# barbararoessle/e2e_multi_view_matching

Measured on AMD Instinct MI355X. Metric: image-pairs/sec @1024 kpts + pose AUC@5/10/20deg vs reference, higher is better.
Workload: dtype f16x2 (fp32 operands carried as 2 fp16 planes hi + 2^-11 lo', 22 significant bits, 3 fp16-MFMA products, fp32 accumulate; same 1e-4 / bit-exact-index parity bar); 1 GPU; configs[1]: tuple_size=2 (1 pair per tuple), 1024 keypoints, 256-dim f32 descriptors, GNN 9x1 = 18 layers, 100 Sinkhorn iters, batch 32 tuples/GPU = 32 pairs/GPU, w8pt pose per pair; pairs_per_gpu=32, global_pairs=32, weights=random init (timed), identity-like for the AUC leg, parallelism=tuple-sharded x1

## Files before the change

e2e_multi_view_matching_amd/csrc/attention_p2w.hip:

```cpp
#include <algorithm>
#include <type_traits>

#include "attention_p2.h"

namespace e2emv {

typedef __attribute__((ext_vector_type(16))) float aw_f32x16;

constexpr int AW_QT = 256;
constexpr int AW_TILEB = 64 * 256;
constexpr int AW_REGB = 2 * AW_TILEB;
constexpr int AW_PART_F = 68;
constexpr float AW_SINV = 1.f / P2_QS, AW_PLOG = 7.f, AW_LIMIT = 60000.f;

__device__ __forceinline__ void aw_wait_q(p2_f16x8 (&q)[2][2][4]) {
    asm volatile("s_waitcnt vmcnt(16)"
                 : "+a"(q[0][0][0]), "+a"(q[0][0][1]), "+a"(q[0][0][2]), "+a"(q[0][0][3]), "+a"(q[0][1][0]), "+a"(q[0][1][1]), "+a"(q[0][1][2]), "+a"(q[0][1][3]),
                   "+a"(q[1][0][0]), "+a"(q[1][0][1]), "+a"(q[1][0][2]), "+a"(q[1][0][3]), "+a"(q[1][1][0]), "+a"(q[1][1][1]), "+a"(q[1][1][2]), "+a"(q[1][1][3])
                 :: "memory");
}

template <int I, int N, class F>
__device__ __forceinline__ void aw_for(F&& f) {
    if constexpr (I < N) {
        f(std::integral_constant<int, I>{});
        aw_for<I + 1, N>(f);
    }
}

__device__ __forceinline__ unsigned aw_cvt_pk(float v0, float v1) {
    const p2_f32x2 vv = {v0, v1};
    return __builtin_bit_cast(unsigned, __builtin_convertvector(vv, p2_f16x2));
}
__device__ __forceinline__ float aw_fma(float a, float b, float c) {
    float d;
    asm volatile("v_fma_f32 %0, %1, %2, %3" : "=v"(d) : "v"(a), "v"(b), "v"(c));
    return d;
}
__device__ __forceinline__ float aw_exp2(float a) {
    float d;
    asm volatile("v_exp_f32 %0, %1" : "=v"(d) : "v"(a));
    return d;
}
__device__ __forceinline__ void aw_acc(float& sum, float a) { asm volatile("v_add_f32 %0, %0, %1" : "+v"(sum) : "v"(a)); }
__device__ __forceinline__ unsigned aw_cvt_pk_v(float v0, float v1) {
    unsigned d;
    asm volatile("v_cvt_pk_f16_f32 %0, %1, %2" : "=v"(d) : "v"(v0), "v"(v1));
    return d;
}
__device__ __forceinline__ unsigned aw_mixlo(unsigned hi, float v0) {
    unsigned lo;
    asm volatile("v_fma_mixlo_f16 %0, %1, -1.0, %2 op_sel_hi:[1,0,0]" : "=v"(lo) : "v"(hi), "v"(v0));
    return lo;
}
__device__ __forceinline__ unsigned aw_mixhi(unsigned lo, unsigned hi, float v1) {
    asm volatile("v_fma_mixhi_f16 %0, %1, -1.0, %2 op_sel:[1,0,0] op_sel_hi:[1,0,0]" : "+v"(lo) : "v"(hi), "v"(v1));
    return lo;
}
__device__ __forceinline__ unsigned aw_lo(unsigned hi, float v0, float v1) {
    unsigned lo;
    asm("v_fma_mixlo_f16 %0, %1, -1.0, %2 op_sel_hi:[1,0,0]\n\tv_fma_mixhi_f16 %0, %1, -1.0, %3 op_sel:[1,0,0] op_sel_hi:[1,0,0]"
        : "=&v"(lo) : "v"(hi), "v"(v0), "v"(v1));
    return lo;
}

__device__ __forceinline__ void aw_mfma_s(aw_f32x16& c, p2_f16x8 a, p2_f16x8 b) {
    asm volatile("v_mfma_f32_32x32x16_f16 %0, %1, %2, %0" : "+v"(c) : "v"(a), "a"(b));
}
__device__ __forceinline__ void aw_mfma_s0(aw_f32x16& c, p2_f16x8 a, p2_f16x8 b) {
    asm volatile("v_mfma_f32_32x32x16_f16 %0, %1, %2, 0" : "=&v"(c) : "v"(a), "a"(b));
}
__device__ __forceinline__ void aw_mfma_sa(aw_f32x16& c, p2_f16x8 a, p2_f16x8 b) {
    asm volatile("v_mfma_f32_32x32x16_f16 %0, %1, %2, %0" : "+v"(c) : "a"(a), "a"(b));
}
__device__ __forceinline__ void aw_mfma_sa0(aw_f32x16& c, p2_f16x8 a, p2_f16x8 b) {
    asm volatile("v_mfma_f32_32x32x16_f16 %0, %1, %2, 0" : "=&v"(c) : "a"(a), "a"(b));
}
__device__ __forceinline__ void aw_mfma_oa(aw_f32x16& c, p2_f16x8 a, p2_u32x4 b) {
    asm volatile("v_mfma_f32_32x32x16_f16 %0, %1, %2, %0" : "+a"(c) : "a"(a), "v"(b));
}
template <int IMM>
__device__ __forceinline__ void aw_read_frag(p2_f16x8& d, unsigned addr) {
    static_assert(IMM >= 0 && IMM < 65536, "ds_read offset: 16 bits");
    asm volatile("ds_read_b128 %0, %1 offset:%2" : "=a"(d) : "v"(addr), "n"(IMM));
}
template <int N>
__device__ __forceinline__ void aw_wait_frag(p2_f16x8 (&f)[4]) {
    asm volatile("s_waitcnt lgkmcnt(%4)" : "+a"(f[0]), "+a"(f[1]), "+a"(f[2]), "+a"(f[3]) : "n"(N));
}
__device__ __forceinline__ void aw_load_q(const char* qp, p2_f16x8 (&q)[2][4]) {
    asm volatile(
        "global_load_dwordx4 %0, %8, off\n\t"
        "global_load_dwordx4 %1, %8, off offset:32\n\t"
        "global_load_dwordx4 %2, %8, off offset:128\n\t"
        "global_load_dwordx4 %3, %8, off offset:160\n\t"
        "global_load_dwordx4 %4, %8, off offset:64\n\t"
        "global_load_dwordx4 %5, %8, off offset:96\n\t"
        "global_load_dwordx4 %6, %8, off offset:192\n\t"
        "global_load_dwordx4 %7, %8, off offset:224"
        : "=&a"(q[0][0]), "=&a"(q[0][1]), "=&a"(q[0][2]), "=&a"(q[0][3]), "=&a"(q[1][0]), "=&a"(q[1][1]), "=&a"(q[1][2]), "=&a"(q[1][3])
        : "v"(qp) : "memory");
}

template <bool HAS_E, bool MULTI = true, bool PART = false>
__global__ __launch_bounds__(256, 1) void attention_p2w_kernel(AttnP2Params p) {
    extern __shared__ __attribute__((aligned(16))) char smem_aw[];

    int lin = blockIdx.x, ks = 0;
    constexpr bool part = PART;
    if constexpr (PART) {
        const int h = blockIdx.x, tpx = (8 * p.gper * p.nq - p.n_full) >> 3;
        ks = (h >> 3) / tpx;
        lin = p.n_full + 8 * ((h >> 3) % tpx) + (h & 7);
    }
    const int xcd = lin & 7, idx = lin >> 3;
    const int g = xcd * p.gper + idx / p.nq;
    if (g >= p.groups) return;
    const int qt = idx % p.nq;
    const int img = g / p.H, head = g % p.H;
    const int b = img / p.T, t = img % p.T;
    if (qt * AW_QT >= p.nv[t]) return;

    const int tid = threadIdx.x, lane = tid & 63;
    const int wave = __builtin_amdgcn_readfirstlane(tid >> 6);
    const int l31 = lane & 31, lh = lane >> 5;
    const unsigned row_b = 8u * (unsigned)p.D;

    int q_row[2];
    bool q_ok[2];
    p2_f16x8 Qf[2][2][4];
#pragma unroll
    for (int a = 0; a < 2; ++a) {
        q_row[a] = qt * AW_QT + wave * 64 + a * 32 + l31;
        q_ok[a] = q_row[a] < p.n_rows;
        const char* qp = reinterpret_cast<const char*>(p.qk) + ((int64_t)img * p.n_rows + (q_ok[a] ? q_row[a] : p.n_rows - 1)) * row_b + head * 256;
        aw_load_q(qp + lh * 16, Qf[a]);
    }
    const int q_blk = __builtin_amdgcn_readfirstlane(((int64_t)img * p.n_rows + min(qt * AW_QT + wave * 64, p.n_rows - 1)) >> 6);
    const int e_q = HAS_E ? p.EQK[q_blk * 8 + head] : 0;

    const int n_src = p.cross ? p.T - 1 : 1;
    auto src_t = [&](int si) __attribute__((always_inline)) { return !p.cross ? t : (si < t ? si : si + 1); };
    int n_tiles = 0;
    for (int si = 0; si < n_src; ++si) n_tiles += (p.nv[src_t(si)] + 63) / 64;
    int t0 = 0;
    if constexpr (PART) {
        t0 = ks * n_tiles / p.n_split;
        n_tiles = (ks + 1) * n_tiles / p.n_split - t0;
        if (n_tiles <= 0) return;
    }
    struct Cur { int si, kt, nv; unsigned kb, vb; int eb; };
    auto cur_src = [&](Cur& c) __attribute__((always_inline)) {
        const int im = b * p.T + src_t(c.si);
        c.kt = 0;
        c.nv = p.nv[src_t(c.si)];
        c.kb = (unsigned)(im * p.n_rows) * row_b;
        c.vb = (unsigned)((im * p.H + head) * 64) * (unsigned)p.n_rows * 4u;
        c.eb = (im * p.n_rows) >> 6;
    };
    auto cur_next = [&](Cur& c) __attribute__((always_inline)) {
        ++c.kt;
        if constexpr (MULTI) {
            if (c.kt * 64 >= c.nv && c.si + 1 < n_src) { ++c.si; cur_src(c); }
        }
    };
    auto cur_init = [&]() __attribute__((always_inline)) {
        Cur c;
        c.si = 0;
        cur_src(c);
        if constexpr (PART)
            for (int i = 0; i < t0; ++i) cur_next(c);
        return c;
    };

    const __amdgpu_buffer_rsrc_t rsK = __builtin_amdgcn_make_buffer_rsrc(const_cast<uint16_t*>(p.qk), 0, (int)p.qk_bytes, 0x00020000);
    const __amdgpu_buffer_rsrc_t rsV = __builtin_amdgcn_make_buffer_rsrc(const_cast<uint16_t*>(p.vt), 0, (int)p.vt_bytes, 0x00020000);
    unsigned k_vo[4], v_vo[4];
#pragma unroll
    for (int i = 0; i < 4; ++i) {
        const int row = 4 * (wave * 4 + i) + (lane >> 4);
        const unsigned c = (unsigned)((lane & 15) ^ (row & 15));
        k_vo[i] = (unsigned)row * row_b + 4u * (unsigned)p.D + (unsigned)head * 256u + c * 16u;
        v_vo[i] = (unsigned)row * (unsigned)p.n_rows * 4u + c * 16u;
    }
    auto k_so = [&](const Cur& c) __attribute__((always_inline)) { return c.kb + (unsigned)c.kt * 64u * row_b; };
    auto v_so = [&](const Cur& c) __attribute__((always_inline)) { return c.vb + (unsigned)c.kt * 256u; };
    auto k_piece = [&](int region, int i, unsigned so) __attribute__((always_inline)) { p2_glds16(rsK, smem_aw + region * AW_REGB + AW_TILEB + (wave * 4 + i) * 1024, k_vo[i], so); };
    auto v_piece = [&](int region, int i, unsigned so) __attribute__((always_inline)) { p2_glds16(rsV, smem_aw + region * AW_REGB + (wave * 4 + i) * 1024, v_vo[i], so); };
    int* const els = reinterpret_cast<int*>(smem_aw + 3 * AW_REGB);
    int ek_mine = 0, ev_mine = 0;
    if (HAS_E && tid < n_tiles) {
        int si = 0, kt = PART ? tid + t0 : tid;
        if constexpr (MULTI) {
            for (; si + 1 < n_src; ++si) {
                const int nt = (p.nv[src_t(si)] + 63) / 64;
                if (kt < nt) break;
                kt -= nt;
            }
        }
        const int blk = (((b * p.T + src_t(si)) * p.n_rows) >> 6) + kt;
        ek_mine = p.EQK[blk * 8 + 4 + head];
        if (p.EVt) ev_mine = p.EVt[blk * 4 + head];
    }
    typedef __attribute__((address_space(3))) const p2_u32x2* lds_pair_t;
    const unsigned els0 = (unsigned)(uintptr_t)(__attribute__((address_space(3))) char*)smem_aw + 3u * AW_REGB;
    auto read_e = [&](int tl) __attribute__((always_inline)) {
        return *reinterpret_cast<lds_pair_t>((uintptr_t)(els0 + 8u * (unsigned)min(tl, n_tiles - 1)));
    };

    const int kz = l31 & 15;
    const unsigned lds0 = (unsigned)(uintptr_t)(__attribute__((address_space(3))) char*)smem_aw;
    unsigned R[4][2];
#pragma unroll
    for (int s = 0; s < 4; ++s)
#pragma unroll
        for (int pl = 0; pl < 2; ++pl)
            R[s][pl] = lds0 + (unsigned)(l31 * 256 + ((((s >> 1) * 8 + pl * 4 + 2 * (s & 1) + lh) ^ kz) << 4));
    typedef __attribute__((address_space(3))) const p2_f16x8* lds_frag_t;
    auto frag = [&](int s, int pl, int imm) __attribute__((always_inline)) { return *reinterpret_cast<lds_frag_t>((uintptr_t)(R[s][pl] + (unsigned)imm)); };

    constexpr int PA[3] = {1, 0, 0};
    constexpr int PB[3] = {0, 1, 0};

    aw_f32x16 O[2][2], S[2][2];
    p2_u32x4 Pf[2][2][4];
#pragma unroll
    for (int a = 0; a < 2; ++a)
#pragma unroll
        for (int d = 0; d < 2; ++d)
#pragma unroll
            for (int r = 0; r < 16; ++r) O[a][d][r] = 0.f;
    float m_run[2] = {-1e30f, -1e30f}, l_run[2] = {0.f, 0.f};
    int e_o = 0;
    bool o_started = false;
    unsigned n_slow = 0;

    auto sm_slow = [&](auto BB, float sinv, int valid) __attribute__((always_inline)) {
        constexpr int B = decltype(BB)::value;
        asm volatile("s_nop 15" : "+v"(S[B][0]), "+v"(S[B][1]), "+a"(O[B][0]), "+a"(O[B][1]));
        if (valid < 64) {
#pragma unroll
            for (int kb = 0; kb < 2; ++kb)
#pragma unroll
                for (int r = 0; r < 16; ++r)
                    if (kb * 32 + (r & 3) + 8 * (r >> 2) + 4 * lh >= valid) S[B][kb][r] = -INFINITY;
        }
        float mx = S[B][0][0];
#pragma unroll
        for (int kb = 0; kb < 2; ++kb)
#pragma unroll
            for (int r = 0; r < 16; ++r) mx = fmaxf(mx, S[B][kb][r]);
        {
            float x = mx, y = mx;
            asm volatile("s_nop 1\n\tv_permlane32_swap_b32 %0, %1\n\ts_nop 1" : "+v"(x), "+v"(y));
            mx = fmaxf(x, y);
        }
        mx *= sinv;
        const float m_new = fmaxf(m_run[B], mx);
        const float alpha = __builtin_amdgcn_exp2f(m_run[B] - m_new);
#pragma unroll
        for (int r = 0; r < 16; ++r) { O[B][0][r] *= alpha; O[B][1][r] *= alpha; }
        const float e0 = AW_PLOG - m_new;
        float ps = 0.f;
#pragma unroll
        for (int k = 0; k < 16; ++k) {
            const int kb = k >> 3, r = 2 * (k & 7), u = 2 * kb + ((k & 7) >> 2), e = k & 3;
            const float p0 = __builtin_amdgcn_exp2f(__builtin_fmaf(S[B][kb][r], sinv, e0));
            const float p1 = __builtin_amdgcn_exp2f(__builtin_fmaf(S[B][kb][r + 1], sinv, e0));
            ps += p0 + p1;
            const P2Pair pr = p2_split_plain(p0, p1);
            Pf[B][0][u][e] = pr.hi; Pf[B][1][u][e] = pr.lo;
        }
        l_run[B] = l_run[B] * alpha + ps;
        m_run[B] = m_new;
        asm volatile("s_nop 4" : "+a"(O[B][0]), "+a"(O[B][1]));
    };

    Cur cK = cur_init(), cV = cur_init(), cS = cur_init();
    int nK = 0, nV = 0;
    auto adv_k = [&]() __attribute__((always_inline)) { if (++nK < n_tiles) cur_next(cK); };
    auto adv_v = [&]() __attribute__((always_inline)) { if (++nV < n_tiles) cur_next(cV); };
    {
        const unsigned so = k_so(cK);
#pragma unroll
        for (int i = 0; i < 4; ++i) k_piece(2, i, so);
        adv_k();
    }
#pragma unroll
    for (int r = 0; r < 2; ++r) {
        const unsigned sov = v_so(cV), sok = k_so(cK);
#pragma unroll
        for (int i = 0; i < 4; ++i) v_piece(r, i, sov);
#pragma unroll
        for (int i = 0; i < 4; ++i) k_piece(r, i, sok);
        adv_v();
        adv_k();
    }
    if (HAS_E && tid < n_tiles) { els[2 * tid] = ek_mine; els[2 * tid + 1] = ev_mine; }
    aw_wait_q(Qf);
    __syncthreads();
    p2_u32x2 e_pair = {0u, 0u};
    if constexpr (HAS_E) e_pair = read_e(0);
#pragma unroll
    for (int s = 0; s < 4; ++s)
#pragma unroll
        for (int pl = 0; pl < 2; ++pl) R[s][pl] += 2 * AW_REGB;
    {
        const float sinv = AW_SINV * p2_exp2i(e_q + __builtin_amdgcn_readfirstlane((int)e_pair[0]));
#pragma unroll
        for (int a = 0; a < 2; ++a)
#pragma unroll
            for (int s = 0; s < 4; ++s) {
                p2_f16x8 kf[2][2];
#pragma unroll
                for (int kb = 0; kb < 2; ++kb)
#pragma unroll
                    for (int pl = 0; pl < 2; ++pl) kf[kb][pl] = frag(s, pl, AW_TILEB + kb * 8192);
#pragma unroll
                for (int q = 0; q < 3; ++q)
#pragma unroll
                    for (int kb = 0; kb < 2; ++kb) {
                        if (s == 0 && q == 0) aw_mfma_s0(S[a][kb], kf[kb][PA[q]], Qf[a][PB[q]][s]);
                        else aw_mfma_s(S[a][kb], kf[kb][PA[q]], Qf[a][PB[q]][s]);
                    }
            }
        asm volatile("s_waitcnt vmcnt(8) lgkmcnt(0)\n\ts_barrier" ::: "memory");
        sm_slow(std::integral_constant<int, 0>{}, sinv, cS.nv - cS.kt * 64);
        if (cS.nv - cS.kt * 64 >= 64) {
            asm volatile("s_nop 15" : "+v"(S[1][0]), "+v"(S[1][1]));
            float mx = S[1][0][0];
#pragma unroll
            for (int kb = 0; kb < 2; ++kb)
#pragma unroll
                for (int r = 0; r < 16; ++r) mx = fmaxf(mx, S[1][kb][r]);
            float x = mx, y = mx;
            asm volatile("s_nop 1\n\tv_permlane32_swap_b32 %0, %1\n\ts_nop 1" : "+v"(x), "+v"(y));
            m_run[1] = fmaxf(x, y) * sinv;
        }
    }
#pragma unroll
    for (int s = 0; s < 4; ++s)
#pragma unroll
        for (int pl = 0; pl < 2; ++pl) R[s][pl] -= 2 * AW_REGB;
    int reg_cur = 0, seg_tile = 0;

    p2_f16x8 FA[8][4];
    auto read_frag = [&](auto GG, auto NN, auto SS, auto KK) __attribute__((always_inline)) {
        constexpr int G = decltype(GG)::value, N = decltype(NN)::value, S = decltype(SS)::value, KPART = decltype(KK)::value;
        constexpr int x = N & 1, pl = N < 2 ? 1 : 0;
        aw_read_frag<KPART * AW_TILEB + x * 8192>(FA[G][N], R[S][pl]);
    };
    aw_for<0, 8>([&](auto II) __attribute__((always_inline)) {
        constexpr int g = decltype(II)::value / 4, n = decltype(II)::value % 4;
        read_frag(std::integral_constant<int, g>{}, std::integral_constant<int, n>{}, std::integral_constant<int, g>{}, std::integral_constant<int, 0>{});
    });

    auto seg = [&](auto AA, auto LL) __attribute__((always_inline)) {
        constexpr int A = decltype(AA)::value, B = 1 - A;
        constexpr bool LAST = decltype(LL)::value;
        constexpr bool HAS_SM = !(LAST && A == 1);
        constexpr int NSLOT = LAST ? 24 : 48, NG = NSLOT / 6;
        constexpr int MPS = LAST ? 2 : 1;

        if (A == 0) {
            if (HAS_E && p.EVt) {
                const int e_v = __builtin_amdgcn_readfirstlane((int)e_pair[1]);
                if (__builtin_expect(o_started && e_v != e_o, 0)) {
                    const float f = e_o - e_v < -126 ? 0.f : p2_exp2i(e_o - e_v);
                    asm volatile("s_nop 15" : "+a"(O[0][0]), "+a"(O[0][1]), "+a"(O[1][0]), "+a"(O[1][1]));
#pragma unroll
                    for (int a = 0; a < 2; ++a)
#pragma unroll
                        for (int r = 0; r < 16; ++r) { O[a][0][r] *= f; O[a][1][r] *= f; }
                    asm volatile("s_nop 4" : "+a"(O[0][0]), "+a"(O[0][1]), "+a"(O[1][0]), "+a"(O[1][1]));
                }
                e_o = e_v;
                o_started = true;
            }
        }
        float sinv = AW_SINV, e0 = 0.f, ps = 0.f;
        int valid = 64;
        if (HAS_SM) {
            if (HAS_E) sinv = AW_SINV * p2_exp2i(e_q + __builtin_amdgcn_readfirstlane((int)e_pair[0]));
            if (HAS_E && A == 0 && !LAST) e_pair = read_e(seg_tile + 1);
            e0 = AW_PLOG - m_run[B];
            valid = cS.nv - cS.kt * 64;
        }
        if (HAS_SM && __builtin_expect(valid < 64, 0)) {
            asm volatile("s_nop 7" : "+v"(S[B][0]), "+v"(S[B][1]));
#pragma unroll
            for (int kb = 0; kb < 2; ++kb)
#pragma unroll
                for (int r = 0; r < 16; ++r)
                    if (kb * 32 + (r & 3) + 8 * (r >> 2) + 4 * lh >= valid) S[B][kb][r] = -INFINITY;
            asm volatile("" : "+v"(S[B][0]), "+v"(S[B][1]));
        }
        bool slow = false;
        float xa[16][2], pa[16][2], psA = 0.f, psB = 0.f, sinv_v = sinv;
        asm volatile("" : "+v"(sinv_v), "+v"(e0));
        unsigned hi_k[16], lo_k[16];
        auto micro = [&](auto MM) __attribute__((always_inline)) {
            constexpr int m = decltype(MM)::value;
            constexpr int k = m / 3, ph = m % 3;
            constexpr int kb = (k & 15) >> 3, r = 2 * (k & 7);
            if constexpr (m == 48) {
                lo_k[15] = aw_mixlo(hi_k[15], pa[15][0]);
            } else if constexpr (m == 49) {
                Pf[B][1][3][3] = aw_mixhi(lo_k[15], hi_k[15], pa[15][1]);
            } else if constexpr (ph == 0) {
                xa[k][0] = aw_fma(S[B][kb][r], sinv_v, e0);
                if constexpr (k > 0) lo_k[k - 1] = aw_mixlo(hi_k[k - 1], pa[k - 1][0]);
                xa[k][1] = aw_fma(S[B][kb][r + 1], sinv_v, e0);
            } else if constexpr (ph == 1) {
                pa[k][0] = aw_exp2(xa[k][0]);
                if constexpr (k > 0) {
                    constexpr int k1 = k - 1, u = 2 * (k1 >> 3) + ((k1 & 7) >> 2), e = k1 & 3;
                    Pf[B][1][u][e] = aw_mixhi(lo_k[k1], hi_k[k1], pa[k1][1]);
                }
                pa[k][1] = aw_exp2(xa[k][1]);
            } else {
                constexpr int u = 2 * (k >> 3) + ((k & 7) >> 2), e = k & 3;
                aw_acc(psA, pa[k][0]);
                hi_k[k] = aw_cvt_pk_v(pa[k][0], pa[k][1]);
                Pf[B][0][u][e] = hi_k[k];
                aw_acc(psB, pa[k][1]);
            }
        };

        unsigned so_v = 0, so_k = 0;
        if (A == 0 && !LAST) {
            so_v = v_so(cV);
            adv_v();
            so_k = k_so(cK);
            adv_k();
        }
        const int reg_ld = reg_cur == 0 ? 2 : reg_cur - 1;

        aw_for<0, NSLOT>([&](auto II) __attribute__((always_inline)) {
            constexpr int i = decltype(II)::value;
            constexpr int gq = i / 6, w = i % 6;
            if constexpr (A == 0 && w == 0) aw_wait_frag<(gq + 1 < NG ? 4 : 0)>(FA[gq]);
            if constexpr (i < 24) {
                constexpr int u = i / 6, q = (i % 6) / 2, db = i % 2;
                aw_mfma_oa(O[A][db], FA[u][db + 2 * (1 - PA[q])], Pf[A][PB[q]][u]);
            } else {
                constexpr int s = (i - 24) / 6, q = (i % 6) / 2, kb = i % 2;
                if constexpr (s == 0 && q == 0) aw_mfma_sa0(S[A][kb], FA[4 + s][kb + 2 * (1 - PA[q])], Qf[A][PB[q]][s]);
                else aw_mfma_sa(S[A][kb], FA[4 + s][kb + 2 * (1 - PA[q])], Qf[A][PB[q]][s]);
            }
            if constexpr (HAS_SM) {
                if constexpr (LAST) {
                    aw_for<0, MPS>([&](auto JJ) __attribute__((always_inline)) { micro(std::integral_constant<int, MPS * i + decltype(JJ)::value>{}); });
                } else if constexpr (i < 9) {
                    constexpr int m0 = i + i / 2 - (i > 0 && i % 2 == 0 ? 1 : 0);
                    micro(std::integral_constant<int, m0>{});
                    if constexpr (i >= 2 && i % 2 == 0) micro(std::integral_constant<int, m0 + 1>{});
                } else if constexpr (i < 46) {
                    micro(std::integral_constant<int, i + 4>{});
                } else if constexpr (i == 46) {
                    ps = psA;
                    aw_acc(ps, psB);
                } else if constexpr (i == 47) {
                    slow = __builtin_amdgcn_ballot_w64(!(ps < AW_LIMIT)) != 0;
                    l_run[B] += slow ? 0.f : ps;
                }
            }
            if constexpr (A == 1 && !LAST && i == 36) {
                asm volatile("s_waitcnt vmcnt(8) lgkmcnt(0)\n\ts_barrier" ::: "memory");
                const unsigned d = reg_cur == 2 ? (unsigned)(-2 * AW_REGB) : (unsigned)AW_REGB;
#pragma unroll
                for (int s = 0; s < 4; ++s)
#pragma unroll
                    for (int pl = 0; pl < 2; ++pl) R[s][pl] += d;
                reg_cur = reg_cur == 2 ? 0 : reg_cur + 1;
            }
            if constexpr (w >= 1 && w <= 4) {
                constexpr int gn = gq + 2;
                constexpr auto N = std::integral_constant<int, w - 1>{};
                if constexpr (A == 0 && gn < NG) {
                    if constexpr (gn < 4) read_frag(std::integral_constant<int, gn>{}, N, std::integral_constant<int, gn>{}, std::integral_constant<int, 0>{});
                    else read_frag(std::integral_constant<int, gn>{}, N, std::integral_constant<int, gn - 4>{}, std::integral_constant<int, 1>{});
                } else if constexpr (A == 1 && !LAST && gn >= NG) {
                    read_frag(std::integral_constant<int, gn - NG>{}, N, std::integral_constant<int, gn - NG>{}, std::integral_constant<int, 0>{});
                }
            }
            if constexpr (A == 0 && !LAST && i < 32 && i % 4 == 1) {
                if constexpr (i < 16) v_piece(reg_ld, i / 4, so_v);
                else k_piece(reg_ld, i / 4 - 4, so_k);
            }
            __builtin_amdgcn_sched_barrier(0);
        });

        if constexpr (HAS_SM && LAST) {
            lo_k[15] = aw_mixlo(hi_k[15], pa[15][0]);
            ps = psA + psB;
            Pf[B][1][3][3] = aw_mixhi(lo_k[15], hi_k[15], pa[15][1]);
            const bool slow = __builtin_amdgcn_ballot_w64(!(ps < AW_LIMIT)) != 0;
            l_run[B] += slow ? 0.f : ps;
            if (__builtin_expect(slow, 0)) {
                sm_slow(std::integral_constant<int, B>{}, sinv, valid);
                ++n_slow;
            }
        }
        if constexpr (HAS_SM && !LAST) {
            if (__builtin_expect(slow, 0)) {
                sm_slow(std::integral_constant<int, B>{}, sinv, valid);
                ++n_slow;
            }
        }
        if (A == 0) cur_next(cS);
    };

    for (int j = 0; j + 1 < n_tiles; ++j) {
        seg_tile = j;
        seg(std::integral_constant<int, 0>{}, std::false_type{});
        seg(std::integral_constant<int, 1>{}, std::false_type{});
    }
    seg(std::integral_constant<int, 0>{}, std::true_type{});
    seg(std::integral_constant<int, 1>{}, std::true_type{});

    asm volatile("s_waitcnt vmcnt(0)" ::: "memory");
    asm volatile("s_nop 15" : "+a"(O[0][0]), "+a"(O[0][1]), "+a"(O[1][0]), "+a"(O[1][1]));
    if constexpr (PART) {
        const int64_t rec = ((int64_t)(lin - p.n_full) * p.n_split + ks) * AW_QT;
        if (lane == 0) p.part_e[rec / 64 + wave] = e_o;
#pragma unroll
        for (int a = 0; a < 2; ++a) {
            const float l_tot = l_run[a] + __shfl_xor(l_run[a], 32);
            float* o = p.part + (rec + wave * 64 + a * 32 + l31) * AW_PART_F;
#pragma unroll
            for (int d = 0; d < 2; ++d)
#pragma unroll
                for (int gq = 0; gq < 4; ++gq)
                    *reinterpret_cast<p2_f32x4*>(o + 32 * d + 8 * gq + 4 * lh) = p2_f32x4{O[a][d][4 * gq], O[a][d][4 * gq + 1], O[a][d][4 * gq + 2], O[a][d][4 * gq + 3]};
            if (lh == 0) { o[64] = m_run[a]; o[65] = l_tot; }
        }
        if (p.stats && n_slow && lane == 0) atomicAdd(p.stats, n_slow);
        return;
    }
    if (p.EO && lane == 0 && q_ok[0]) p.EO[(((int64_t)img * p.n_rows + q_row[0]) >> 6) * 4 + head] = e_o;
#pragma unroll
    for (int a = 0; a < 2; ++a) {
        const float l_tot = l_run[a] + __shfl_xor(l_run[a], 32);
        const float inv = 1.f / (l_tot * P2_VS);
        uint16_t* op = p.out + p2_index((int64_t)img * p.n_rows + q_row[a], head * 64, p.D) + 8 * lh;
#pragma unroll
        for (int d = 0; d < 2; ++d)
#pragma unroll
            for (int kp = 0; kp < 2; ++kp) {
                const int r0 = 8 * kp, r1 = 8 * kp + 4;
                const P2Pair x0 = p2_split_scaled(O[a][d][r0] * inv, O[a][d][r0 + 1] * inv), x1 = p2_split_scaled(O[a][d][r0 + 2] * inv, O[a][d][r0 + 3] * inv);
                const P2Pair y0 = p2_split_scaled(O[a][d][r1] * inv, O[a][d][r1 + 1] * inv), y1 = p2_split_scaled(O[a][d][r1 + 2] * inv, O[a][d][r1 + 3] * inv);
                const auto h0 = __builtin_amdgcn_permlane32_swap(x0.hi, y0.hi, false, false), h1 = __builtin_amdgcn_permlane32_swap(x1.hi, y1.hi, false, false);
                const auto l0 = __builtin_amdgcn_permlane32_swap(x0.lo, y0.lo, false, false), l1 = __builtin_amdgcn_permlane32_swap(x1.lo, y1.lo, false, false);
                uint16_t* o = op + d * 64 + kp * 16;
                if (q_ok[a]) {
                    *reinterpret_cast<p2_u32x4*>(o) = p2_u32x4{h0[0], h1[0], h0[1], h1[1]};
                    *reinterpret_cast<p2_u32x4*>(o + 32) = p2_u32x4{l0[0], l1[0], l0[1], l1[1]};
                }
            }
    }
    if (p.stats && n_slow && lane == 0) atomicAdd(p.stats, n_slow);
}

__global__ __launch_bounds__(1024) void attention_p2w_combine(AttnP2Params p) {
    const int item = blockIdx.x, lin = p.n_full + item;
    const int xcd = lin & 7, idx = lin >> 3;
    const int g = xcd * p.gper + idx / p.nq;
    if (g >= p.groups) return;
    const int qt = idx % p.nq, img = g / p.H, head = g % p.H, t = img % p.T;
    if (qt * AW_QT >= p.nv[t]) return;
    const int n_src = p.cross ? p.T - 1 : 1;
    int n_tiles = 0;
    for (int si = 0; si < n_src; ++si) n_tiles += (p.nv[!p.cross ? t : (si < t ? si : si + 1)] + 63) / 64;
    const int q = threadIdx.x >> 2, dq = (threadIdx.x & 3) * 16;
    const int row = qt * AW_QT + q;
    float m = -3.0e38f;
    int e = -1000;
    for (int k = 0; k < p.n_split; ++k) {
        if ((k + 1) * n_tiles / p.n_split - k * n_tiles / p.n_split <= 0) continue;
        const int64_t rec = ((int64_t)item * p.n_split + k) * AW_QT;
        m = fmaxf(m, p.part[(rec + q) * AW_PART_F + 64]);
        e = max(e, p.part_e[rec / 64 + (q >> 6)]);
    }
    float acc[16], l = 0.f;
#pragma unroll
    for (int i = 0; i < 16; ++i) acc[i] = 0.f;
    for (int k = 0; k < p.n_split; ++k) {
        if ((k + 1) * n_tiles / p.n_split - k * n_tiles / p.n_split <= 0) continue;
        const int64_t rec = ((int64_t)item * p.n_split + k) * AW_QT;
        const float* o = p.part + (rec + q) * AW_PART_F;
        const int ek = p.part_e[rec / 64 + (q >> 6)];
        const float a = __builtin_amdgcn_exp2f(o[64] - m);
        const float ae = a * (ek - e < -126 ? 0.f : p2_exp2i(ek - e));
        l += a * o[65];
#pragma unroll
        for (int i = 0; i < 16; i += 4) {
            const p2_f32x4 v = *reinterpret_cast<const p2_f32x4*>(o + dq + i);
            acc[i] += ae * v[0]; acc[i + 1] += ae * v[1]; acc[i + 2] += ae * v[2]; acc[i + 3] += ae * v[3];
        }
    }
    if (row >= p.n_rows) return;
    if (p.EO && (threadIdx.x & 255) == 0) p.EO[(((int64_t)img * p.n_rows + row) >> 6) * 4 + head] = e;
    const float inv = 1.f / (l * P2_VS);
    uint16_t* op = p.out + p2_index((int64_t)img * p.n_rows + row, head * 64 + dq, p.D);
#pragma unroll
    for (int h = 0; h < 2; ++h) {
        p2_u32x4 hi, lo;
#pragma unroll
        for (int i = 0; i < 4; ++i) {
            const P2Pair pr = p2_split_scaled(acc[8 * h + 2 * i] * inv, acc[8 * h + 2 * i + 1] * inv);
            hi[i] = pr.hi; lo[i] = pr.lo;
        }
        *reinterpret_cast<p2_u32x4*>(op + 8 * h) = hi;
        *reinterpret_cast<p2_u32x4*>(op + 8 * h + 32) = lo;
    }
}

int launch_attention_p2w(e2emv_ctx* ctx, AttnP2Params& p, int n_valid, hipStream_t s) {
    p.nq = (n_valid + AW_QT - 1) / AW_QT;
    if (int rc = ensure_flags(ctx)) return rc;
    p.stats = ctx->d_flags + 5;
    const size_t lds = 3 * AW_REGB + 2048;
    const bool multi = p.cross && p.T > 2;
    const void* fn = p.EQK ? (multi ? reinterpret_cast<const void*>(attention_p2w_kernel<true, true>) : reinterpret_cast<const void*>(attention_p2w_kernel<true, false>))
                           : (multi ? reinterpret_cast<const void*>(attention_p2w_kernel<false, true>) : reinterpret_cast<const void*>(attention_p2w_kernel<false, false>));
    if (int rc = ensure_dynamic_lds(ctx, fn, lds)) return rc;
    void* args[] = {&p};
    const int n_items = 8 * p.gper * p.nq, cus = std::max(8, ctx->num_cus / 8 * 8);
    const int r = n_items % cus;
    const int min_tiles = attn_min_tiles(p, 64);
    p.n_full = n_items;
    p.n_split = 1;
    p.part = nullptr;
    p.part_e = nullptr;
    if (ctx->attn_key_split && r > 0 && 2 * r <= cus && r % 8 == 0) {
        const int k = std::min(std::min(cus / r, 8), min_tiles);
        if (k >= 2) {
            const size_t n_rec = (size_t)r * k * AW_QT;
            const size_t need = n_rec * AW_PART_F * sizeof(float) + (n_rec / 64) * sizeof(int);
            if (need > ctx->attn_part_bytes) {
                if (ctx->d_attn_part) { E2EMV_HIP(ctx, hipStreamSynchronize(s)); (void)hipFree(ctx->d_attn_part); ctx->d_attn_part = nullptr; ctx->attn_part_bytes = 0; }
                E2EMV_HIP(ctx, hipMalloc((void**)&ctx->d_attn_part, need));
                ctx->attn_part_bytes = need;
            }
            p.n_full = n_items - r;
            p.n_split = k;
            p.part = ctx->d_attn_part;
            p.part_e = reinterpret_cast<int*>(ctx->d_attn_part + n_rec * AW_PART_F);
        }
    }
    if (p.n_full > 0) {
        E2EMV_HIP(ctx, hipLaunchKernel(fn, dim3(p.n_full), dim3(256), args, lds, s));
        E2EMV_CHECK_LAUNCH(ctx, "attention_p2w_kernel");
    }
    if (p.n_split > 1) {
        const void* fp = p.EQK ? (multi ? reinterpret_cast<const void*>(attention_p2w_kernel<true, true, true>) : reinterpret_cast<const void*>(attention_p2w_kernel<true, false, true>))
                               : (multi ? reinterpret_cast<const void*>(attention_p2w_kernel<false, true, true>) : reinterpret_cast<const void*>(attention_p2w_kernel<false, false, true>));
        if (int rc = ensure_dynamic_lds(ctx, fp, lds)) return rc;
        E2EMV_HIP(ctx, hipLaunchKernel(fp, dim3((n_items - p.n_full) * p.n_split), dim3(256), args, lds, s));
        E2EMV_CHECK_LAUNCH(ctx, "attention_p2w_kernel (parts)");
        hipLaunchKernelGGL(attention_p2w_combine, dim3(n_items - p.n_full), dim3(1024), 0, s, p);
        E2EMV_CHECK_LAUNCH(ctx, "attention_p2w_combine");
    }
    return E2EMV_OK;
}

}
```

Before: 3479 pairs/s.

## Stage Q through LDS and interleave prologue K/V loads with first-tile MFMAs

Q fragments are no longer fetched with direct global loads into AGPRs. They are brought into LDS with buffer-to-LDS copies that use the same swizzle as K, then read back with ds_read. The prologue loads of the first two V/K regions are deferred and spread among the MFMAs of the first QK tile, and K fragments for that tile are double-buffered across s so reads overlap compute. LDS usage grows by three tiles to hold the per-wave Q images, and the ordering now depends on hand-placed sched_barriers and waitcnt counts.

```diff
diff --git a/e2e_multi_view_matching_amd/csrc/attention_p2w.hip b/e2e_multi_view_matching_amd/csrc/attention_p2w.hip
--- a/e2e_multi_view_matching_amd/csrc/attention_p2w.hip
+++ b/e2e_multi_view_matching_amd/csrc/attention_p2w.hip
@@ -10,11 +10,14 @@
 constexpr int AW_QT = 256;
 constexpr int AW_TILEB = 64 * 256;
 constexpr int AW_REGB = 2 * AW_TILEB;
+constexpr int AW_ELS = 3 * AW_REGB;
+constexpr int AW_QIMG = AW_ELS + 2048;
+constexpr int AW_LDS = AW_QIMG + 3 * AW_TILEB;
 constexpr int AW_PART_F = 68;
 constexpr float AW_SINV = 1.f / P2_QS, AW_PLOG = 7.f, AW_LIMIT = 60000.f;
 
-__device__ __forceinline__ void aw_wait_q(p2_f16x8 (&q)[2][2][4]) {
-    asm volatile("s_waitcnt vmcnt(16)"
+__device__ __forceinline__ void aw_wait_q_k0(p2_f16x8 (&q)[2][2][4]) {
+    asm volatile("s_waitcnt vmcnt(0) lgkmcnt(0)\n\ts_barrier"
                  : "+a"(q[0][0][0]), "+a"(q[0][0][1]), "+a"(q[0][0][2]), "+a"(q[0][0][3]), "+a"(q[0][1][0]), "+a"(q[0][1][1]), "+a"(q[0][1][2]), "+a"(q[0][1][3]),
                    "+a"(q[1][0][0]), "+a"(q[1][0][1]), "+a"(q[1][0][2]), "+a"(q[1][0][3]), "+a"(q[1][1][0]), "+a"(q[1][1][1]), "+a"(q[1][1][2]), "+a"(q[1][1][3])
                  :: "memory");
@@ -88,20 +91,6 @@
 __device__ __forceinline__ void aw_wait_frag(p2_f16x8 (&f)[4]) {
     asm volatile("s_waitcnt lgkmcnt(%4)" : "+a"(f[0]), "+a"(f[1]), "+a"(f[2]), "+a"(f[3]) : "n"(N));
 }
-__device__ __forceinline__ void aw_load_q(const char* qp, p2_f16x8 (&q)[2][4]) {
-    asm volatile(
-        "global_load_dwordx4 %0, %8, off\n\t"
-        "global_load_dwordx4 %1, %8, off offset:32\n\t"
-        "global_load_dwordx4 %2, %8, off offset:128\n\t"
-        "global_load_dwordx4 %3, %8, off offset:160\n\t"
-        "global_load_dwordx4 %4, %8, off offset:64\n\t"
-        "global_load_dwordx4 %5, %8, off offset:96\n\t"
-        "global_load_dwordx4 %6, %8, off offset:192\n\t"
-        "global_load_dwordx4 %7, %8, off offset:224"
-        : "=&a"(q[0][0]), "=&a"(q[0][1]), "=&a"(q[0][2]), "=&a"(q[0][3]), "=&a"(q[1][0]), "=&a"(q[1][1]), "=&a"(q[1][2]), "=&a"(q[1][3])
-        : "v"(qp) : "memory");
-}
-
 template <bool HAS_E, bool MULTI = true, bool PART = false>
 __global__ __launch_bounds__(256, 1) void attention_p2w_kernel(AttnP2Params p) {
     extern __shared__ __attribute__((aligned(16))) char smem_aw[];
@@ -133,11 +122,24 @@
     for (int a = 0; a < 2; ++a) {
         q_row[a] = qt * AW_QT + wave * 64 + a * 32 + l31;
         q_ok[a] = q_row[a] < p.n_rows;
-        const char* qp = reinterpret_cast<const char*>(p.qk) + ((int64_t)img * p.n_rows + (q_ok[a] ? q_row[a] : p.n_rows - 1)) * row_b + head * 256;
-        aw_load_q(qp + lh * 16, Qf[a]);
     }
     const int q_blk = __builtin_amdgcn_readfirstlane(((int64_t)img * p.n_rows + min(qt * AW_QT + wave * 64, p.n_rows - 1)) >> 6);
-    const int e_q = HAS_E ? p.EQK[q_blk * 8 + head] : 0;
+    const int e_q_v = HAS_E ? p.EQK[q_blk * 8 + head] : 0;
+    const unsigned q_img = wave == 0 ? 2u * AW_REGB : (unsigned)(AW_QIMG + (wave - 1) * AW_TILEB);
+    {
+        const __amdgpu_buffer_rsrc_t rsQ = __builtin_amdgcn_make_buffer_rsrc(const_cast<uint16_t*>(p.qk), 0, (int)p.qk_bytes, 0x00020000);
+        const unsigned so = (unsigned)(img * p.n_rows) * row_b;
+        asm volatile("" ::: "memory");
+#pragma unroll
+        for (int i = 0; i < 16; ++i) {
+            const int rl = 4 * i + (lane >> 4);
+            const int row = min(qt * AW_QT + wave * 64 + rl, p.n_rows - 1);
+            const unsigned c = (unsigned)((lane & 15) ^ (rl & 15));
+            p2_glds16(rsQ, smem_aw + q_img + i * 1024, (unsigned)row * row_b + (unsigned)head * 256u + c * 16u, so);
+        }
+        asm volatile("" ::: "memory");
+    }
+    const int e_q = __builtin_amdgcn_readfirstlane(e_q_v);
 
     const int n_src = p.cross ? p.T - 1 : 1;
     auto src_t = [&](int si) __attribute__((always_inline)) { return !p.cross ? t : (si < t ? si : si + 1); };
@@ -187,7 +189,7 @@
     auto v_so = [&](const Cur& c) __attribute__((always_inline)) { return c.vb + (unsigned)c.kt * 256u; };
     auto k_piece = [&](int region, int i, unsigned so) __attribute__((always_inline)) { p2_glds16(rsK, smem_aw + region * AW_REGB + AW_TILEB + (wave * 4 + i) * 1024, k_vo[i], so); };
     auto v_piece = [&](int region, int i, unsigned so) __attribute__((always_inline)) { p2_glds16(rsV, smem_aw + region * AW_REGB + (wave * 4 + i) * 1024, v_vo[i], so); };
-    int* const els = reinterpret_cast<int*>(smem_aw + 3 * AW_REGB);
+    int* const els = reinterpret_cast<int*>(smem_aw + AW_ELS);
     int ek_mine = 0, ev_mine = 0;
     if (HAS_E && tid < n_tiles) {
         int si = 0, kt = PART ? tid + t0 : tid;
@@ -203,7 +205,7 @@
         if (p.EVt) ev_mine = p.EVt[blk * 4 + head];
     }
     typedef __attribute__((address_space(3))) const p2_u32x2* lds_pair_t;
-    const unsigned els0 = (unsigned)(uintptr_t)(__attribute__((address_space(3))) char*)smem_aw + 3u * AW_REGB;
+    const unsigned els0 = (unsigned)(uintptr_t)(__attribute__((address_space(3))) char*)smem_aw + (unsigned)AW_ELS;
     auto read_e = [&](int tl) __attribute__((always_inline)) {
         return *reinterpret_cast<lds_pair_t>((uintptr_t)(els0 + 8u * (unsigned)min(tl, n_tiles - 1)));
     };
@@ -286,44 +288,64 @@
         for (int i = 0; i < 4; ++i) k_piece(2, i, so);
         adv_k();
     }
+    unsigned so_v01[2], so_k12[2];
 #pragma unroll
     for (int r = 0; r < 2; ++r) {
-        const unsigned sov = v_so(cV), sok = k_so(cK);
-#pragma unroll
-        for (int i = 0; i < 4; ++i) v_piece(r, i, sov);
-#pragma unroll
-        for (int i = 0; i < 4; ++i) k_piece(r, i, sok);
+        so_v01[r] = v_so(cV);
+        so_k12[r] = k_so(cK);
         adv_v();
         adv_k();
     }
     if (HAS_E && tid < n_tiles) { els[2 * tid] = ek_mine; els[2 * tid + 1] = ev_mine; }
-    aw_wait_q(Qf);
-    __syncthreads();
+#pragma unroll
+    for (int s = 0; s < 4; ++s)
+#pragma unroll
+        for (int pl = 0; pl < 2; ++pl) R[s][pl] += q_img;
+    asm volatile("s_waitcnt vmcnt(4)" ::: "memory");
+    aw_for<0, 16>([&](auto II) __attribute__((always_inline)) {
+        constexpr int a = decltype(II)::value >> 3, pl = (decltype(II)::value >> 2) & 1, s = decltype(II)::value & 3;
+        aw_read_frag<a * 8192>(Qf[a][pl][s], R[s][pl]);
+    });
+    aw_wait_q_k0(Qf);
     p2_u32x2 e_pair = {0u, 0u};
     if constexpr (HAS_E) e_pair = read_e(0);
 #pragma unroll
     for (int s = 0; s < 4; ++s)
 #pragma unroll
-        for (int pl = 0; pl < 2; ++pl) R[s][pl] += 2 * AW_REGB;
+        for (int pl = 0; pl < 2; ++pl) R[s][pl] += 2 * AW_REGB - q_img;
     {
         const float sinv = AW_SINV * p2_exp2i(e_q + __builtin_amdgcn_readfirstlane((int)e_pair[0]));
-#pragma unroll
-        for (int a = 0; a < 2; ++a)
-#pragma unroll
-            for (int s = 0; s < 4; ++s) {
-                p2_f16x8 kf[2][2];
+        p2_f16x8 kf[2][2][2];
+#pragma unroll
+        for (int kb = 0; kb < 2; ++kb)
+#pragma unroll
+            for (int pl = 0; pl < 2; ++pl) kf[0][kb][pl] = frag(0, pl, AW_TILEB + kb * 8192);
+#pragma unroll
+        for (int s = 0; s < 4; ++s) {
+            if (s < 3) {
 #pragma unroll
                 for (int kb = 0; kb < 2; ++kb)
 #pragma unroll
-                    for (int pl = 0; pl < 2; ++pl) kf[kb][pl] = frag(s, pl, AW_TILEB + kb * 8192);
+                    for (int pl = 0; pl < 2; ++pl) kf[(s + 1) & 1][kb][pl] = frag(s + 1, pl, AW_TILEB + kb * 8192);
+            }
+            __builtin_amdgcn_sched_barrier(0);
+#pragma unroll
+            for (int a = 0; a < 2; ++a)
 #pragma unroll
                 for (int q = 0; q < 3; ++q)
 #pragma unroll
                     for (int kb = 0; kb < 2; ++kb) {
-                        if (s == 0 && q == 0) aw_mfma_s0(S[a][kb], kf[kb][PA[q]], Qf[a][PB[q]][s]);
-                        else aw_mfma_s(S[a][kb], kf[kb][PA[q]], Qf[a][PB[q]][s]);
+                        if (s == 0 && q == 0) aw_mfma_s0(S[a][kb], kf[s & 1][kb][PA[q]], Qf[a][PB[q]][s]);
+                        else aw_mfma_s(S[a][kb], kf[s & 1][kb][PA[q]], Qf[a][PB[q]][s]);
+                        const int slot = s * 12 + a * 6 + q * 2 + kb;
+                        if (slot % 3 == 1) {
+                            const int n = slot / 3, r = n >> 3, i = n & 3;
+                            if ((n & 4) == 0) v_piece(r, i, so_v01[r]);
+                            else k_piece(r, i, so_k12[r]);
+                        }
+                        __builtin_amdgcn_sched_barrier(0);
                     }
-            }
+        }
         asm volatile("s_waitcnt vmcnt(8) lgkmcnt(0)\n\ts_barrier" ::: "memory");
         sm_slow(std::integral_constant<int, 0>{}, sinv, cS.nv - cS.kt * 64);
         if (cS.nv - cS.kt * 64 >= 64) {
@@ -621,7 +643,7 @@
     p.nq = (n_valid + AW_QT - 1) / AW_QT;
     if (int rc = ensure_flags(ctx)) return rc;
     p.stats = ctx->d_flags + 5;
-    const size_t lds = 3 * AW_REGB + 2048;
+    const size_t lds = AW_LDS;
     const bool multi = p.cross && p.T > 2;
     const void* fn = p.EQK ? (multi ? reinterpret_cast<const void*>(attention_p2w_kernel<true, true>) : reinterpret_cast<const void*>(attention_p2w_kernel<true, false>))
                            : (multi ? reinterpret_cast<const void*>(attention_p2w_kernel<false, true>) : reinterpret_cast<const void*>(attention_p2w_kernel<false, false>));
```

New measurement: 3533 pairs/s, median of 6. 1.5% higher.
